# ajaayc/Probability-of-Collision-for-Safe-Planning

Measured on AMD Instinct MI355X. Metric: particle-waypoint evals/s (GMM+collision), higher is better.
Workload: dtype f64

## Files before the change

### probability-of-collision-for-safe-planning_amd/csrc/pocs_collide.h

```cpp
#pragma once
#include "pocs_math.h"

#define POCS_OBS_STRIDE 8
#define POCS_MAX_OBSTACLES 64

struct pocs_footprint { double dx, dy, hx, hy; };

POCS_HD void pocs_prepare_obstacle(const double box5[5], const pocs_footprint* fp, double* rec) {
  double sn, cs;
  pocs_sincos(box5[4], &sn, &cs);
  const double rr = sqrt(fp->hx * fp->hx + fp->hy * fp->hy);
  rec[0] = box5[0]; rec[1] = box5[1];
  rec[2] = cs; rec[3] = sn;
  rec[4] = box5[2]; rec[5] = box5[3];
  rec[6] = (box5[2] * fabs(cs) + box5[3] * fabs(sn)) + rr;
  rec[7] = (box5[2] * fabs(sn) + box5[3] * fabs(cs)) + rr;
}

POCS_HD bool pocs_box_margins(double dx, double dy, double sn, double cs, double rx, double ry, double hx, double hy,
                              double cr, double sr, double e1, double e2) {
  const double m3 = fabs(e1) - (hx + fma(rx, fabs(cr), ry * fabs(sr)));
  const double m4 = fabs(e2) - (hy + fma(rx, fabs(sr), ry * fabs(cr)));
  if (fmax(m3, m4) > 0.0) return false;
#if defined(__HIP_DEVICE_COMPILE__)
  asm volatile("; footprint axes");
#endif
  const double d1 = fma(dx, cs, dy * sn);
  const double d2 = fma(dy, cs, -(dx * sn));
  const double m1 = fabs(d1) - (rx + fma(hx, fabs(cr), hy * fabs(sr)));
  const double m2 = fabs(d2) - (ry + fma(hx, fabs(sr), hy * fabs(cr)));
  return !(fmax(m1, m2) > 0.0);
}

POCS_HD bool pocs_box_narrow(double px, double py, double sn, double cs, double rx, double ry,
                             const double* o) {
  const double dx = o[0] - px;
  const double dy = o[1] - py;
  const double ax = o[2], ay = o[3], hx = o[4], hy = o[5];
  if (ax == 1.0 && ay == 0.0)
    return pocs_box_margins(dx, dy, sn, cs, rx, ry, hx, hy, cs, sn, dx, dy);
  return pocs_box_margins(dx, dy, sn, cs, rx, ry, hx, hy,
                          fma(cs, ax, sn * ay),
                          fma(sn, ax, -(cs * ay)),
                          fma(dx, ax, dy * ay),
                          fma(dy, ax, -(dx * ay)));
}

POCS_HD bool pocs_box_hit(double px, double py, double sn, double cs, double rx, double ry,
                          const double* o) {
  if (fabs(o[0] - px) > o[6] || fabs(o[1] - py) > o[7]) return false;
  return pocs_box_narrow(px, py, sn, cs, rx, ry, o);
}

POCS_HD bool pocs_pose_collides(double x, double y, double th, const pocs_footprint* fp,
                                const double* obs, int M, const pocs_tables* T, const pocs_vconst* V = nullptr) {
  if (M <= 0) return false;
  double sn, cs;
  pocs_sincos_tab(th, T, &sn, &cs, V);
  double px = x, py = y;
  if (!(fp->dx == 0.0 && fp->dy == 0.0)) {
#if defined(__HIP_DEVICE_COMPILE__)
    asm volatile("; offset footprint");
#endif
    px = x + fma(cs, fp->dx, -(sn * fp->dy));
    py = y + fma(sn, fp->dx, cs * fp->dy);
  }
  bool hit = false;
  for (int m = 0; m < M; ++m)
    if (pocs_box_hit(px, py, sn, cs, fp->hx, fp->hy, obs + m * POCS_OBS_STRIDE)) hit = true;
  return hit;
}

template <bool EAGER = false>
POCS_HD void pocs_pair_collides(const double x[2], const double y[2], const double th[2], const pocs_footprint* fp,
                                const double* obs, int M, const pocs_tables* T, const pocs_vconst* V, bool hit[2]) {
  hit[0] = false; hit[1] = false;
  if (M <= 0) return;
  double sn[2], cs[2], px[2], py[2];
#if defined(__HIP_DEVICE_COMPILE__)
#pragma unroll
#endif
  for (int h = 0; h < 2; ++h) {
    pocs_sincos_tab(th[h], T, &sn[h], &cs[h], V);
    px[h] = x[h]; py[h] = y[h];
  }
  if (!(fp->dx == 0.0 && fp->dy == 0.0)) {
#if defined(__HIP_DEVICE_COMPILE__)
    asm volatile("; offset footprint");
#endif
    for (int h = 0; h < 2; ++h) {
      px[h] = x[h] + fma(cs[h], fp->dx, -(sn[h] * fp->dy));
      py[h] = y[h] + fma(sn[h], fp->dx, cs[h] * fp->dy);
    }
  }
  for (int m = 0; m < M; ++m) {
    const double* o = obs + m * POCS_OBS_STRIDE;
#if defined(__HIP_DEVICE_COMPILE__)
    double rec[POCS_OBS_STRIDE];
    if (EAGER) {
#pragma unroll
      for (int q = 0; q < POCS_OBS_STRIDE; ++q) rec[q] = o[q];
      asm volatile("" : "+v"(rec[0]), "+v"(rec[1]), "+v"(rec[2]), "+v"(rec[3]), "+v"(rec[4]), "+v"(rec[5]), "+v"(rec[6]), "+v"(rec[7]));
      o = rec;
    }
#pragma unroll
#endif
    for (int h = 0; h < 2; ++h)
      if (pocs_box_hit(px[h], py[h], sn[h], cs[h], fp->hx, fp->hy, o)) hit[h] = true;
  }
}

template <class Each>
POCS_HD bool pocs_pose_collides_each(double x, double y, double th, const pocs_footprint* fp, const double* obs, int M,
                                     const pocs_tables* T, Each each, const pocs_vconst* V = nullptr) {
  if (M <= 0) return false;
  double sn, cs;
  pocs_sincos_tab(th, T, &sn, &cs, V);
  double px = x, py = y;
  if (!(fp->dx == 0.0 && fp->dy == 0.0)) {
#if defined(__HIP_DEVICE_COMPILE__)
    asm volatile("; offset footprint");
#endif
    px = x + fma(cs, fp->dx, -(sn * fp->dy));
    py = y + fma(sn, fp->dx, cs * fp->dy);
  }
  bool hit = false;
  for (int m = 0; m < M; ++m) {
    const bool t = pocs_box_hit(px, py, sn, cs, fp->hx, fp->hy, obs + m * POCS_OBS_STRIDE);
    if (t) hit = true;
    each(m, t);
  }
  return hit;
}

template <bool EAGER = false, class Each>
POCS_HD void pocs_pair_collides_each(const double x[2], const double y[2], const double th[2], const pocs_footprint* fp,
                                     const double* obs, int M, const pocs_tables* T, const pocs_vconst* V, bool hit[2], Each each) {
  hit[0] = false; hit[1] = false;
  if (M <= 0) return;
  double sn[2], cs[2], px[2], py[2];
#if defined(__HIP_DEVICE_COMPILE__)
#pragma unroll
#endif
  for (int h = 0; h < 2; ++h) {
    pocs_sincos_tab(th[h], T, &sn[h], &cs[h], V);
    px[h] = x[h]; py[h] = y[h];
  }
  if (!(fp->dx == 0.0 && fp->dy == 0.0)) {
#if defined(__HIP_DEVICE_COMPILE__)
    asm volatile("; offset footprint");
#endif
    for (int h = 0; h < 2; ++h) {
      px[h] = x[h] + fma(cs[h], fp->dx, -(sn[h] * fp->dy));
      py[h] = y[h] + fma(sn[h], fp->dx, cs[h] * fp->dy);
    }
  }
  for (int m = 0; m < M; ++m) {
    const double* o = obs + m * POCS_OBS_STRIDE;
#if defined(__HIP_DEVICE_COMPILE__)
    double rec[POCS_OBS_STRIDE];
    if (EAGER) {
#pragma unroll
      for (int q = 0; q < POCS_OBS_STRIDE; ++q) rec[q] = o[q];
      asm volatile("" : "+v"(rec[0]), "+v"(rec[1]), "+v"(rec[2]), "+v"(rec[3]), "+v"(rec[4]), "+v"(rec[5]), "+v"(rec[6]), "+v"(rec[7]));
      o = rec;
    }
#pragma unroll
#endif
    for (int h = 0; h < 2; ++h) {
      const bool t = pocs_box_hit(px[h], py[h], sn[h], cs[h], fp->hx, fp->hy, o);
      if (t) hit[h] = true;
      each(m, h, t);
    }
  }
}

POCS_HD bool pocs_footprint_extent_is_radius(double phi, double lo, double hi) {
  const double PI = 3.14159265358979323846, INV_PI = 0.318309886183790671538;
  if (!(hi - lo < PI)) return true;
  for (int sgn = -1; sgn <= 1; sgn += 2) {
    const double s = sgn * phi;
    if (ceil((lo - s) * INV_PI) <= floor((hi - s) * INV_PI)) return true;
  }
  return false;
}
POCS_HD double pocs_footprint_extent_end(double rx, double ry, double t) {
  double sn, cs;
  pocs_sincos(t, &sn, &cs);
  return fma(rx, fabs(cs), ry * fabs(sn));
}
POCS_HD double pocs_footprint_extent_of_ends(double rr, double fa, double fb) {
  return fmin(rr, fmax(fa, fb) * (1.0 + 1e-9) + 1e-12);
}
POCS_HD double pocs_footprint_extent_pre(double rx, double ry, double rr, double phi, double lo, double hi) {
  if (pocs_footprint_extent_is_radius(phi, lo, hi)) return rr;
  const double fa = pocs_footprint_extent_end(rx, ry, lo);
  const double fb = pocs_footprint_extent_end(rx, ry, hi);
  return pocs_footprint_extent_of_ends(rr, fa, fb);
}
POCS_HD double pocs_footprint_extent(double rx, double ry, double lo, double hi) {
  return pocs_footprint_extent_pre(rx, ry, sqrt(rx * rx + ry * ry), atan2(ry, rx), lo, hi);
}
```

### probability-of-collision-for-safe-planning_amd/csrc/pocs_dev_gmm.hpp

```cpp

template <bool OC> struct gmm_oc_smem {};
template <> struct gmm_oc_smem<true> {
  unsigned occ[2][POCS_MAX_OBSTACLES];
  int oci[2][POCS_MAX_OBSTACLES];
};
template <int K, int TB, bool OC = false>
struct gmm_smem : gmm_oc_smem<OC> {
  static constexpr int NC = K * POCS_NMOM;
  static constexpr int NW = TB / 64;
  static constexpr int SUB = POCS_GMM_SUB;
  alignas(16) pocs_tables tab;
  alignas(16) double keep[2][POCS_MAX_OBSTACLES * POCS_OBS_STRIDE];
  alignas(16) double par[2][K * POCS_PARAM_STRIDE];
  alignas(16) double tr[NW][POCS_FLUSH_ROWS][POCS_FLUSH_PITCH];
  alignas(16) double slot[SUB][NW][POCS_UNIT_SUMS];
  double xtra[2][NW][K][POCS_UNIT_SUMS];
  int kf[SUB][NW];
  int xj[2][NW][K];
  unsigned long long seed[2];
  int nkeep[2];
  int last[2];
  static_assert(sizeof(double) * NW * POCS_FLUSH_ROWS * POCS_FLUSH_PITCH >= sizeof(double) * POCS_MAX_OBSTACLES * POCS_OBS_STRIDE,
                "the obstacle table is staged in the transpose scratch");
  static_assert(NW * POCS_FLUSH_ROWS * POCS_FLUSH_PITCH >= 16 * NC, "the closer's staging rows live in the transpose scratch");
  static_assert(SUB * NW * POCS_UNIT_SUMS >= POCS_ADV_SCRATCH(K) + POCS_SPEC_SCRATCH(K), "the advance's scratch lives in the slots");
  __device__ __forceinline__ double* obs() { return &tr[0][0][0]; }
  __device__ __forceinline__ double* stage() { return &tr[0][0][0]; }
  __device__ __forceinline__ double* adv() { return &slot[0][0][0]; }
  __device__ __forceinline__ double* spec() { return &slot[0][0][0] + POCS_ADV_SCRATCH(K); }
};

__device__ __forceinline__ double oct_sum(double s) {
  s += dpp_f64<0xB1>(s);
  s += dpp_f64<0x4E>(s);
  s += dpp_f64<0x141>(s);
  return s;
}

template <int K, int TB, bool OC>
__device__ __forceinline__ void flush_unit(gmm_smem<K, TB, OC>& sm, const int wave, const int lane, const int rb, const int tl,
                                           const int k, bool& first, double (&acc)[9], int& nfree) {
  double* const T = &sm.tr[wave][0][0];
  double* const dst = first ? &sm.slot[tl][wave][0] : &sm.xtra[rb][wave][k][0];
  const int j = lane >> 3, q = lane & 7;
#pragma unroll
  for (int pass = 0; pass < 2; ++pass) {
    const int nv = pass == 0 ? 5 : 4, v0 = pass == 0 ? 0 : 5;
#pragma unroll
    for (int i = 0; i < nv; ++i) T[i * POCS_FLUSH_PITCH + lane] = acc[v0 + i];
    __builtin_amdgcn_fence(__ATOMIC_RELEASE, "wavefront");
    __builtin_amdgcn_wave_barrier();
    double s = 0.0;
    if (j < nv) {
      const double* p = &T[j * POCS_FLUSH_PITCH + 8 * q];
      s = p[0]; s += p[1]; s += p[2]; s += p[3]; s += p[4]; s += p[5]; s += p[6]; s += p[7];
    }
    s = oct_sum(s);
    if (j < nv && q == 0) dst[1 + v0 + j] = s;
    __builtin_amdgcn_fence(__ATOMIC_RELEASE, "wavefront");
    __builtin_amdgcn_wave_barrier();
  }
  if (lane == 0) {
    dst[0] = (double)nfree;
    if (first) sm.kf[tl][wave] = k; else sm.xj[rb][wave][k] = tl;
  }
#pragma unroll
  for (int i = 0; i < 9; ++i) acc[i] = 0.0;
  nfree = 0;
  first = false;
}

template <int K>
__device__ __forceinline__ void gmm_reach(const pocs_footprint& fp, const double fp_rr, const double fp_phi, const int lane, const double* par,
                                          pocs_reach& rc, double& ext_x, double& ext_y) {
  pocs_world_reach_box(par, K, fp, rc);
  const double tlo = rc.tlo, thi = rc.thi;
  const double HALF_PI = 1.57079632679489661923;
  const double end_t = ((lane & 1) ? thi : tlo) - ((lane & 2) ? HALF_PI : 0.0);
  const double end_f = pocs_footprint_extent_end(fp.hx, fp.hy, end_t);
  ext_x = pocs_footprint_extent_is_radius(fp_phi, tlo, thi) ? fp_rr
        : pocs_footprint_extent_of_ends(fp_rr, lane_value(end_f, 0), lane_value(end_f, 1));
  ext_y = pocs_footprint_extent_is_radius(fp_phi, tlo - HALF_PI, thi - HALF_PI) ? fp_rr
        : pocs_footprint_extent_of_ends(fp_rr, lane_value(end_f, 2), lane_value(end_f, 3));
}
template <int K, int TB, bool OC>
__device__ __forceinline__ void gmm_cull(const pocs_gmm_launch& a, gmm_smem<K, TB, OC>& sm, const int rb, const int lane, const double* par) {
  const pocs_footprint fp = a.fp;
  const int M = a.M;
  const double* const obs = sm.obs();
  double xlo = 1e300, xhi = -1e300, ylo = 1e300, yhi = -1e300, tlo = 1e300, thi = -1e300;
#pragma unroll
  for (int k = 0; k < K; ++k) {
    const double* p = &par[k * POCS_PARAM_STRIDE];
    const double ex = 6.67 * fabs(p[3]), ey = 6.67 * (fabs(p[4]) + fabs(p[5])), et = 6.67 * (fabs(p[6]) + fabs(p[7]) + fabs(p[8]));
    xlo = fmin(xlo, p[0] - ex); xhi = fmax(xhi, p[0] + ex);
    ylo = fmin(ylo, p[1] - ey); yhi = fmax(yhi, p[1] + ey);
    tlo = fmin(tlo, p[2] - et); thi = fmax(thi, p[2] + et);
  }
  const double pad = sqrt(fp.dx * fp.dx + fp.dy * fp.dy) + 1e-6;
  xlo -= pad; xhi += pad; ylo -= pad; yhi += pad;
  tlo -= 1e-9 * (1.0 + fabs(tlo)); thi += 1e-9 * (1.0 + fabs(thi));
  const double HALF_PI = 1.57079632679489661923;
  const double end_t = ((lane & 1) ? thi : tlo) - ((lane & 2) ? HALF_PI : 0.0);
  const double end_f = pocs_footprint_extent_end(fp.hx, fp.hy, end_t);
  const double ext_x = pocs_footprint_extent_is_radius(a.fp_phi, tlo, thi) ? a.fp_rr
                     : pocs_footprint_extent_of_ends(a.fp_rr, lane_value(end_f, 0), lane_value(end_f, 1));
  const double ext_y = pocs_footprint_extent_is_radius(a.fp_phi, tlo - HALF_PI, thi - HALF_PI) ? a.fp_rr
                     : pocs_footprint_extent_of_ends(a.fp_rr, lane_value(end_f, 2), lane_value(end_f, 3));
  bool keep = false;
  double bx = 0.0, by = 0.0;
  if (lane < M) {
    const double* o = &obs[lane * POCS_OBS_STRIDE];
    bx = fmin(o[6], fma(o[4], fabs(o[2]), o[5] * fabs(o[3])) * (1.0 + 1e-12) + ext_x);
    by = fmin(o[7], fma(o[4], fabs(o[3]), o[5] * fabs(o[2])) * (1.0 + 1e-12) + ext_y);
    keep = !(o[0] - bx > xhi || o[0] + bx < xlo || o[1] - by > yhi || o[1] + by < ylo);
  }
  const unsigned long long mask = __ballot(keep);
  if (keep) {
    const int pos = __popcll(mask & ((1ull << lane) - 1ull));
#pragma unroll
    for (int j = 0; j < 6; ++j) sm.keep[rb][pos * POCS_OBS_STRIDE + j] = obs[lane * POCS_OBS_STRIDE + j];
    sm.keep[rb][pos * POCS_OBS_STRIDE + 6] = bx;
    sm.keep[rb][pos * POCS_OBS_STRIDE + 7] = by;
    if constexpr (OC) sm.oci[rb][pos] = lane;
  }
  if constexpr (OC) sm.occ[rb][lane] = 0u;
  if (lane == 0) sm.nkeep[rb] = __popcll(mask);
}

template <int K, bool STORE, int TB, bool LONE_PRE = false, bool OC = false>
__device__ __forceinline__ void gmm_units(const pocs_gmm_launch& a, gmm_smem<K, TB, OC>& sm, const int w, const int r0,
                                          const int ta, const int tb, const double* zpre = nullptr, const int npre = 0) {
  const pocs_tables* const s_tab = &sm.tab;
  const int tid = threadIdx.x, lane = tid & 63;
  const int wave = __builtin_amdgcn_readfirstlane(tid >> 6);
  const pocs_footprint fp = a.fp;
  const int vs_mask = (1 << a.vs_shift) - 1;
  double acc[9];
  int nfree = 0;
#pragma unroll
  for (int j = 0; j < 9; ++j) acc[j] = 0.0;
  const int count = (int)a.count;
  const int npairs = (count + 1) >> 1;
  const uint64_t pair0 = (uint64_t)(a.first >> 1);
  const double first_d = (double)a.first;
  const int wave_first = 128 * wave;
  const int prio_slot = (TB >= 512 ? (wave >> 2) : 0) + (TB >= 512 ? 2 : 1) * (int)((blockIdx.x >> 8) & 3u);
  int prio_it = prio_slot;
  int rb = -1, nkeep = 0, kcur = 0, kw = 0;
  const double* s_par = nullptr;
  const double* s_keep = nullptr;
  uint64_t seed = 0;
  double cumn[K > 1 ? K - 1 : 1];
  double *xr = nullptr, *yr = nullptr, *tr = nullptr;
  int16_t* fr = nullptr;
  int seg_end = 0;
  POCS_VCONST(vc_);
  const pocs_vconst* const vc = &vc_;

  int it_unit = 0;
  auto iteration = [&](auto whole_tag, const int base, const int tl, bool& first) __attribute__((always_inline)) {
    constexpr bool WHOLE = decltype(whole_tag)::value;
    switch (prio_it++ & 3) {
      case 0: __builtin_amdgcn_s_setprio(0); break;
      case 1: __builtin_amdgcn_s_setprio(1); break;
      case 2: __builtin_amdgcn_s_setprio(2); break;
      default: __builtin_amdgcn_s_setprio(3); break;
    }
    const int lp = base + tid;
    const bool live = WHOLE || lp < npairs;
    double zz[2][3];
    uint32_t spare[2];
    uint64_t seed_it = seed;
#if defined(__HIP_DEVICE_COMPILE__)
    asm volatile("" : "+s"(seed_it));
#endif
    bool drawn = false;
    if constexpr (LONE_PRE) {
      if (it_unit < npre) {
        const double* z = zpre + (size_t)it_unit * 6 * TB + tid;
#pragma unroll
        for (int q = 0; q < 3; ++q) { zz[0][q] = z[q * TB]; zz[1][q] = z[(3 + q) * TB]; }
        drawn = true;
        ++it_unit;
      }
    }
    if (!drawn) {
      POCS_TUNE_NORMALS(pocs_normal3_pair(seed_it, pair0 + (uint64_t)(unsigned)lp, (uint32_t)w, POCS_STREAM_GMM, s_tab, zz[0], zz[1], &spare[0], &spare[1], vc));
    }
    const int i0 = 2 * lp;
    const bool two = WHOLE || (live && (i0 + 1) < count);
    double xs[2], ys[2], ts[2];
    bool hits[2];
    int ks[2];
#pragma unroll
    for (int h = 0; h < 2; ++h) {
      int k = kw;
      if (!WHOLE) {
        const double gidx = (first_d + (double)i0) + (double)h;
        k = 0;
#pragma unroll
        for (int j = 0; j < K - 1; ++j) k += (cumn[j] <= gidx) ? 1 : 0;
      }
      const double* p = &s_par[k * POCS_PARAM_STRIDE];
      xs[h] = fma(p[3], zz[h][0], p[0]);
      ys[h] = fma(p[5], zz[h][1], fma(p[4], zz[h][0], p[1]));
      ts[h] = fma(p[8], zz[h][2], fma(p[7], zz[h][1], fma(p[6], zz[h][0], p[2])));
      ks[h] = k;
    }
    POCS_TUNE_COLLIDE_STATS();
    if constexpr (OC) {
      unsigned* const occ = sm.occ[rb];
      pocs_pair_collides_each<LONE_PRE>(xs, ys, ts, &fp, s_keep, nkeep, s_tab, vc, hits, [&](const int m, const int h, const bool t) {
        const unsigned long long b = __ballot(t && (h == 0 ? live : two));
        if (b != 0ull && lane == (int)__builtin_ctzll(b))
          __hip_atomic_fetch_add(&occ[m], (unsigned)__popcll(b), __ATOMIC_RELAXED, __HIP_MEMORY_SCOPE_WORKGROUP);
      });
    } else {
    POCS_TUNE_COLLIDE(pocs_pair_collides<LONE_PRE>(xs, ys, ts, &fp, s_keep, nkeep, s_tab, vc, hits));
    }
    if constexpr (POCS_TUNE_SKIP_MOMENTS) { POCS_TUNE_MOMENTS_ALT(); } else {
    if (WHOLE) {
#pragma unroll
      for (int h = 0; h < 2; ++h) {
        nfree += __popcll(__ballot(!hits[h]));
        if (!hits[h]) {
          const double x = xs[h], y = ys[h], t = ts[h];
          acc[0] += x; acc[1] += y; acc[2] += t;
          acc[3] = fma(x, x, acc[3]); acc[4] = fma(x, y, acc[4]); acc[5] = fma(x, t, acc[5]);
          acc[6] = fma(y, y, acc[6]); acc[7] = fma(y, t, acc[7]); acc[8] = fma(t, t, acc[8]);
        }
      }
    } else {
      const unsigned long long live_mask = __ballot(live);
      const int klo = live_mask ? __builtin_amdgcn_readlane(ks[0], (int)__builtin_ctzll(live_mask)) : K;
      const int khi = __ballot(two) == ~0ull ? __builtin_amdgcn_readlane(ks[1], 63) : K - 1;
#pragma unroll
      for (int kk = 0; kk < K; ++kk) {
        if (kk < klo || kk > khi) continue;
        if (kk != kcur) { flush_unit(sm, wave, lane, rb, tl, kcur, first, acc, nfree); kcur = kk; }
#pragma unroll
        for (int h = 0; h < 2; ++h) {
          const bool sel = (h == 0 ? live : two) && ks[h] == kk;
          const bool cnt = sel && !hits[h];
          nfree += __popcll(__ballot(cnt));
          const double ind = cnt ? 1.0 : 0.0;
          const double xm = ind * xs[h], ym = ind * ys[h], tm = ind * ts[h];
          acc[0] += xm; acc[1] += ym; acc[2] += tm;
          acc[3] = fma(xm, xs[h], acc[3]); acc[4] = fma(xm, ys[h], acc[4]); acc[5] = fma(xm, ts[h], acc[5]);
          acc[6] = fma(ym, ys[h], acc[6]); acc[7] = fma(ym, ts[h], acc[7]); acc[8] = fma(tm, ts[h], acc[8]);
        }
      }
    }
    }
    if (STORE && live) {
      const size_t ub = 2 * (size_t)(unsigned)base;
      const int fl = (hits[0] ? 1 : 0) | ((two && hits[1]) ? 0x10000 : 0);
      store16_nt(xr + ub, 16u * (unsigned)tid, (v2d){xs[0], xs[1]});
      store16_nt(yr + ub, 16u * (unsigned)tid, (v2d){ys[0], ys[1]});
      store16_nt(tr + ub, 16u * (unsigned)tid, (v2d){ts[0], ts[1]});
      store4_nt(fr + ub, 4u * (unsigned)tid, fl);
    }
  };

  auto lookup = [&](const int l0) __attribute__((always_inline)) {
    const double g0 = first_d + (double)l0;
    int kk = 0;
#pragma unroll
    for (int q = 0; q < K - 1; ++q) kk += (cumn[q] <= g0) ? 1 : 0;
    kw = __builtin_amdgcn_readfirstlane(kk);
    double e = (double)count;
    if (kw < K - 1) e = fmin(e, s_par[kw * POCS_PARAM_STRIDE + 9] - first_d);
    seg_end = __builtin_amdgcn_readfirstlane((int)e);
  };
  for (int t = ta; t < tb; ++t) {
    const int tl = t - ta;
    const int r = t >> a.vs_shift, j = t & vs_mask;
    if (r - r0 != rb) {
      rb = r - r0;
      s_par = sm.par[rb]; s_keep = sm.keep[rb];
      nkeep = __builtin_amdgcn_readfirstlane(sm.nkeep[rb]);
      seed = (uint64_t)uniform64((long long)sm.seed[rb]);
#pragma unroll
      for (int q = 0; q < K - 1; ++q) cumn[q] = s_par[q * POCS_PARAM_STRIDE + 9];
      xr = a.x + (size_t)r * a.sample_stride;
      yr = a.y + (size_t)r * a.sample_stride;
      tr = a.th + (size_t)r * a.sample_stride;
      fr = a.flags + (size_t)r * a.sample_stride;
      seg_end = 0;
    }
    const int c_begin = (int)(((long long)j * a.chunks) >> a.vs_shift);
    const int c_end = (int)(((long long)(j + 1) * a.chunks) >> a.vs_shift);
    bool first = true;
    it_unit = (t == ta) ? 0 : npre;
    const int end = c_end * TB;
    int base = c_begin * TB;
    if (2 * base + wave_first + 128 > seg_end) lookup(2 * base + wave_first);
    kcur = kw;
    while (base < end) {
      int l0 = 2 * base + wave_first;
      if (l0 + 128 > seg_end) lookup(l0);
      if (l0 + 128 <= seg_end) {
        if (kw != kcur) { flush_unit(sm, wave, lane, rb, tl, kcur, first, acc, nfree); kcur = kw; }
        do {
          iteration(std::true_type{}, base, tl, first);
          base += TB;
          l0 += 2 * TB;
        } while (base < end && l0 + 128 <= seg_end);
      } else {
        iteration(std::false_type{}, base, tl, first);
        base += TB;
      }
    }
    __builtin_amdgcn_s_setprio(3);
    flush_unit(sm, wave, lane, rb, tl, kcur, first, acc, nfree);
  }
}

template <int K, int TB, bool OC>
__device__ __forceinline__ void gmm_emit_rows(const pocs_gmm_launch& a, gmm_smem<K, TB, OC>& sm, const int r0, const int ta, const int tb) {
  constexpr int NC = K * POCS_NMOM, NW = TB / 64;
  for (int i = threadIdx.x; i < (tb - ta) * NC; i += TB) {
    const int tl = i / NC, c = i - tl * NC, k = c / POCS_NMOM, col = c - k * POCS_NMOM;
    const int rb = ((ta + tl) >> a.vs_shift) - r0;
    double v = 0.0;
    if (col != 1) {
      const int s = col == 0 ? 0 : col - 1;
      double ps[NW], px[NW];
      int kf[NW], xj[NW];
#pragma unroll
      for (int u = 0; u < NW; ++u) { kf[u] = sm.kf[tl][u]; xj[u] = sm.xj[rb][u][k]; ps[u] = sm.slot[tl][u][s]; px[u] = sm.xtra[rb][u][k][s]; }
#pragma unroll
      for (int u = 0; u < NW; ++u) {
        const double p = kf[u] == k ? ps[u] : (xj[u] == tl ? px[u] : 0.0);
        v = (u == 0) ? p : v + p;
      }
    }
    store_wt(&a.partial[(size_t)(ta + tl) * NC + c], v);
  }
}

template <int K, int NT>
struct close_rows {
  static constexpr int NC = K * POCS_NMOM, G = 16, ITEMS = G * NC, RPI = POCS_GMM_MAX_VS / G;
  double v[2][RPI];
  __device__ __forceinline__ void request(const double* src, const int S, const int i0) {
#pragma unroll
    for (int t = 0; t < 2; ++t) {
      const int i = i0 + t * NT, g = i / NC, c = i - g * NC;
#pragma unroll
      for (int u = 0; u < RPI; ++u) {
        const int q = g + u * G;
        v[t][u] = (i < ITEMS && q < S) ? load_wt(&src[(size_t)q * NC + c]) : 0.0;
      }
    }
  }
  __device__ __forceinline__ void pin() {
    static_assert(RPI % 4 == 0, "four values per statement");
#pragma unroll
    for (int t = 0; t < 2; ++t)
#pragma unroll
      for (int u = 0; u < RPI; u += 4) asm volatile("" : "+v"(v[t][u]), "+v"(v[t][u + 1]), "+v"(v[t][u + 2]), "+v"(v[t][u + 3]));
  }
  __device__ __forceinline__ void reduce(double* stage, const int S, const int i0) const {
#pragma unroll
    for (int t = 0; t < 2; ++t) {
      const int i = i0 + t * NT, g = i / NC;
      double sum = 0.0;
#pragma unroll
      for (int u = 0; u < RPI; ++u) if (g + u * G < S) sum += v[t][u];
      if (i < ITEMS) stage[i] = sum;
    }
  }
};
template <int K>
__device__ __forceinline__ const double* close_rows_of(const pocs_gmm_launch& a, const double* rows, const int r) {
  return rows + (size_t)r * (1 << a.vs_shift) * (K * POCS_NMOM);
}
template <int K, int NT, bool REQUESTED = false>
__device__ __forceinline__ void gmm_close_sums(const pocs_gmm_launch& a, const int w, const int r, const double* s_par,
                                               double* stage, double* tot, const int tid,
                                               const double* rows, const bool store, close_rows<K, NT>& cr) {
  constexpr int NC = K * POCS_NMOM, G = 16, ITEMS = G * NC, nthreads = NT;
  const int S = 1 << a.vs_shift;
  const double* src = close_rows_of<K>(a, rows, r);
  for (int i0 = tid; i0 < ITEMS; i0 += 2 * NT) {
    if (!(REQUESTED && i0 == tid)) cr.request(src, S, i0);
    requests_issued();
    cr.pin();
    cr.reduce(stage, S, i0);
  }
  __syncthreads();
  for (int c = tid; c < NC; c += nthreads) {
    double v = stage[c];
    const int ng = S < G ? S : G;
    for (int g = 1; g < ng; ++g) v += stage[g * NC + c];
    tot[c] = v;
  }
  __syncthreads();
  const double lo = (double)a.first, hi = (double)(a.first + a.count);
  for (int k = tid; k < K; k += nthreads) {
    const double c0 = (k == 0) ? 0.0 : s_par[(k - 1) * POCS_PARAM_STRIDE + 9];
    const double c1 = (k == K - 1) ? (double)a.n_total : s_par[k * POCS_PARAM_STRIDE + 9];
    const double n_k = fmax(0.0, fmin(c1, hi) - fmax(c0, lo));
    tot[k * POCS_NMOM + 1] = n_k - tot[k * POCS_NMOM];
  }
  __syncthreads();
  if (store) for (int c = tid; c < NC; c += nthreads) a.moments[((size_t)w * a.nruns + r) * NC + c] = tot[c];
}

template <int K, bool STORE, int TB, bool LONE, bool RISK, bool TREE = false, bool OC = false, bool WORLD = false>
__device__ __forceinline__ void gmm_step_block(const pocs_gmm_launch a) {
  typedef gmm_smem<K, TB, OC> smem_t;
  static_assert(!(WORLD && (LONE || TREE || OC)), "a large world: the ticket form of a batch or of plans, no per-box counts");
  static_assert(!WORLD || TB == POCS_MAX_OBSTACLES * POCS_OBS_STRIDE, "one element of a run's kept records per thread");
  static_assert(!(LONE && RISK), "the lone form closes in its heads: a call under a risk bound takes the ticket form");
  static_assert(!(TREE && (LONE || STORE)), "a tree's levels take the ticket form and store no samples");
  constexpr int SUB = smem_t::SUB, NW = smem_t::NW;
  __shared__ smem_t sm;
  __shared__ double s_zpre[LONE ? POCS_LONE_PRE * 6 * TB : 2];
  int npre = 0;
  const int tid = threadIdx.x;
  const int w = a.waypoint;
  const int wr = TREE ? 0 : w;
  const int t_lo = a.run_lo << a.vs_shift, t_hi = (a.run_lo + a.run_cnt) << a.vs_shift;
  const int bx = (int)blockIdx.x;
  const int t0_all = t_lo + bx * a.upb;
  const int t1_all = (t0_all + a.upb < t_hi) ? t0_all + a.upb : t_hi;
  const int r0_all = t0_all >> a.vs_shift, r1_all = (t1_all - 1) >> a.vs_shift;
  int t0 = t0_all, t1 = t1_all, r0 = r0_all, r1 = r1_all;
  POCS_STAMP_BEGIN();
  constexpr int PS = K * POCS_PARAM_STRIDE;
  static_assert(POCS_MAX_OBSTACLES * POCS_OBS_STRIDE <= TB, "one obstacle element per thread");
  static_assert(2 * PS <= TB, "one sampler parameter per thread (two runs)");
  static_assert(POCS_ADV_STAGE_MAX <= 4 * TB, "the advance's inputs in one batch");
  double tabv[table_regs<TB>::N];
  request_tables<TB>(a.tables, tid, tabv);
  double obs_elem = 0.0;
  if constexpr (!WORLD) obs_elem = tid < a.M * POCS_OBS_STRIDE ? a.env->obs[tid] : 0.0;
  if (LONE && w > 0) {
    const bool out = blockIdx.x == 0;
    const adv_ptrs ap = advance_ptrs(a, K, w, r0, sm.adv());
    double advv[4];
    advance_request(ap, false, tid, TB, advv);
    const double parv = tid < PS ? a.param[((size_t)r0 * a.W + (w - 1)) * PS + tid] : 0.0;
    const unsigned long long seedv = a.hdr[r0].seed;
    close_rows<K, TB> cr;
    cr.request(close_rows_of<K>(a, a.partial_prev, r0), 1 << a.vs_shift, tid);
    requests_issued();
    commit_tables<TB>(&sm.tab, tid, tabv);
    advance_commit(ap, false, tid, TB, advv);
    if (tid < PS) sm.par[1][tid] = parv;
    for (int j = tid; j < 2 * NW * K; j += TB) (&sm.xj[0][0][0])[j] = -1;
    if (tid == 0) sm.seed[0] = seedv;
    double* const l_mom = ap.l_mom;
    gmm_close_sums<K, TB, true>(a, w - 1, r0, sm.par[1], sm.stage(), l_mom, tid, a.partial_prev, out, cr);
    POCS_STAMP(5);
    if (tid < a.M * POCS_OBS_STRIDE) sm.obs()[tid] = obs_elem;
    const int j0 = t0 & ((1 << a.vs_shift) - 1);
    const int cb0 = (int)(((long long)j0 * a.chunks) >> a.vs_shift), ce0 = (int)(((long long)(j0 + 1) * a.chunks) >> a.vs_shift);
    npre = (ce0 - cb0) < POCS_LONE_PRE ? (ce0 - cb0) : POCS_LONE_PRE;
    auto draw_ahead = [&]() __attribute__((always_inline)) {
      POCS_VCONST(vc_);
      const uint64_t seed = seedv;
      const uint64_t pair0 = (uint64_t)(a.first >> 1);
      for (int it = 0; it < npre; ++it)
        for (int l = tid - 128; l < TB; l += TB - 128) {
          double za[3], zb[3];
          uint32_t sa, sb;
          pocs_normal3_pair(seed, pair0 + (uint64_t)(unsigned)((cb0 + it) * TB + l), (uint32_t)w, POCS_STREAM_GMM, &sm.tab, za, zb, &sa, &sb, &vc_);
          double* z = s_zpre + (size_t)it * 6 * TB + l;
#pragma unroll
          for (int q = 0; q < 3; ++q) { z[q * TB] = za[q]; z[(3 + q) * TB] = zb[q]; }
        }
    };
    auto cull_early = [&]() __attribute__((always_inline)) { gmm_cull(a, sm, 0, tid - 64, ap.l_par); };
    if (tid < 128) __builtin_amdgcn_s_setprio(3);
    advance_block(a, K, w, r0, sm.adv(), sm.spec(), true, tid, TB, true, out, draw_ahead, cull_early);
    if (tid < 128) __builtin_amdgcn_s_setprio(0);
    __syncthreads();
    POCS_STAMP(6);
    POCS_STAMP_COUNT(14);
    const double* const l_par = advance_ptrs(a, K, w, r0, sm.adv()).l_par;
    for (int j = tid; j < PS; j += TB) sm.par[0][j] = l_par[j];
  } else {
    const int rp = tid / PS, jp = tid - rp * PS;
    const double parv = tid < (r1 - r0 + 1) * PS ? load_wt(&a.param[((size_t)(r0 + rp) * a.W + wr) * PS + jp]) : 0.0;
    const unsigned long long seedv = tid <= r1 - r0 ? a.hdr[r0 + tid].seed : 0ull;
    double keptv[2] = {0.0, 0.0};
    int reachv[2] = {0, 0};
    if constexpr (WORLD) {
#pragma unroll
      for (int q = 0; q < 2; ++q) {
        const int rq = r0_all + q <= r1_all ? r0_all + q : r1_all;
        keptv[q] = load_wt(&a.kept[(size_t)rq * (POCS_MAX_OBSTACLES * POCS_OBS_STRIDE) + tid]);
        reachv[q] = __hip_atomic_load(&a.reach[(size_t)rq * a.W + wr], __ATOMIC_RELAXED, __HIP_MEMORY_SCOPE_AGENT);
      }
    }
    auto commit_world = [&](const int shift) __attribute__((always_inline)) {
      if constexpr (WORLD) {
#pragma unroll
        for (int q = 0; q < 2; ++q) {
          const int rb = q - shift;
          if (q <= r1_all - r0_all && rb >= 0 && rb <= r1 - r0) {
            const int n = reachv[q] < POCS_MAX_OBSTACLES ? reachv[q] : POCS_MAX_OBSTACLES;
            if (tid < n * POCS_OBS_STRIDE) sm.keep[rb][tid] = keptv[q];
            if (tid == 0) sm.nkeep[rb] = n;
          }
        }
      }
    };
    if constexpr (RISK) {
      const unsigned s0 = __hip_atomic_load(&a.stop[r0_all], __ATOMIC_RELAXED, __HIP_MEMORY_SCOPE_AGENT);
      const unsigned s1 = __hip_atomic_load(&a.stop[r1_all], __ATOMIC_RELAXED, __HIP_MEMORY_SCOPE_AGENT);
      requests_issued();
      const bool dead0 = __builtin_amdgcn_readfirstlane((int)s0) != 0, dead1 = __builtin_amdgcn_readfirstlane((int)s1) != 0;
      if (dead0 && dead1) return;
      int shift = 0;
      if (dead0) { shift = 1; r0 = r1_all; t0 = r1_all << a.vs_shift; }
      else if (dead1) { r1 = r0_all; t1 = r1_all << a.vs_shift; }
      commit_tables<TB>(&sm.tab, tid, tabv);
      if (tid < a.M * POCS_OBS_STRIDE) sm.obs()[tid] = obs_elem;
      if (tid < (r1_all - r0_all + 1) * PS && rp >= shift && rp - shift <= r1 - r0) sm.par[rp - shift][jp] = parv;
      for (int j = tid; j < 2 * NW * K; j += TB) (&sm.xj[0][0][0])[j] = -1;
      if (tid <= r1_all - r0_all && tid >= shift && tid - shift <= r1 - r0) sm.seed[tid - shift] = seedv;
      commit_world(shift);
    } else {
    requests_issued();
    commit_tables<TB>(&sm.tab, tid, tabv);
    if (tid < a.M * POCS_OBS_STRIDE) sm.obs()[tid] = obs_elem;
    if (tid < (r1 - r0 + 1) * PS) sm.par[rp][jp] = parv;
    for (int j = tid; j < 2 * NW * K; j += TB) (&sm.xj[0][0][0])[j] = -1;
    if (tid <= r1 - r0) sm.seed[tid] = seedv;
    commit_world(0);
    }
  }
  __syncthreads();
  if constexpr (!WORLD) {
  if (!(LONE && w > 0)) {
    if (tid < 64) gmm_cull(a, sm, 0, tid, sm.par[0]);
    else if (tid < 128 && r1 > r0) gmm_cull(a, sm, 1, tid - 64, sm.par[1]);
    __syncthreads();
  }
  }
  POCS_STAMP(0);
  for (int ta = t0; ta < t1; ta += SUB) {
    const int tb = (ta + SUB < t1) ? ta + SUB : t1;
    gmm_units<K, STORE, TB, LONE, OC>(a, sm, w, r0, ta, tb, s_zpre, ta == t0 ? npre : 0);
    POCS_STAMP(1);
    __syncthreads();
    POCS_STAMP(2);
    gmm_emit_rows(a, sm, r0, ta, tb);
    if (tb < t1) {
      __syncthreads();
      for (int j = tid; j < 2 * NW * K; j += TB) (&sm.xj[0][0][0])[j] = -1;
      __syncthreads();
    }
  }
  if constexpr (OC) {
    const int rb = tid >> 6, j = tid & 63;
// ... 196 lines not shown
```

### probability-of-collision-for-safe-planning_amd/csrc/pocs_tuning.h

```cpp
#ifndef POCS_TUNING_HOOKS
#define POCS_TUNING_HOOKS

#if defined(POCS_STAMPS)
__device__ unsigned long long g_stamps[24 * 256];
#define POCS_STAMP_AT(i) (&g_stamps[(i) + 24 * (blockIdx.x & 255)])
#define POCS_STAMP_BEGIN() unsigned long long last_ = wall_clock64(); if (threadIdx.x == 0) atomicAdd(POCS_STAMP_AT(15), 1ull)
#define POCS_STAMP(i) do { if (threadIdx.x == 0) { const unsigned long long n_ = wall_clock64(); atomicAdd(POCS_STAMP_AT(i), n_ - last_); last_ = n_; } } while (0)
#define POCS_STAMP_COUNT(i) do { if (threadIdx.x == 0) atomicAdd(POCS_STAMP_AT(i), 1ull); } while (0)
#define POCS_ADV_STAMP_BEGIN() unsigned long long t_ = wall_clock64()
#define POCS_ADV_STAMP(i) do { if (tid == 0) { const unsigned long long n_ = wall_clock64(); atomicAdd(POCS_STAMP_AT(i), n_ - t_); t_ = n_; } } while (0)
#define POCS_TUNE_COLLIDE_STATS() do { bool pass_ = false; \
    for (int m_ = 0; m_ < nkeep; ++m_) { const double* o_ = s_keep + m_ * POCS_OBS_STRIDE; \
      for (int h_ = 0; h_ < 2; ++h_) pass_ = pass_ || (fabs(o_[0] - xs[h_]) <= o_[6] && fabs(o_[1] - ys[h_]) <= o_[7]); } \
    const unsigned long long b_ = __ballot(pass_); \
    bool own_ = false; { const double* p_ = &s_par[ks[0] * POCS_PARAM_STRIDE]; const double ex_ = 6.67 * fabs(p_[3]), ey_ = 6.67 * (fabs(p_[4]) + fabs(p_[5])); \
      for (int m_ = 0; m_ < nkeep; ++m_) { const double* o_ = s_keep + m_ * POCS_OBS_STRIDE; \
        own_ = own_ || (fabs(o_[0] - p_[0]) <= o_[6] + ex_ && fabs(o_[1] - p_[1]) <= o_[7] + ey_); } } \
    const unsigned long long c_ = __ballot(own_); \
    if ((threadIdx.x & 63) == 0) { atomicAdd(POCS_STAMP_AT(16), 1ull); if (nkeep > 0) atomicAdd(POCS_STAMP_AT(17), 1ull); if (b_) atomicAdd(POCS_STAMP_AT(18), 1ull); \
      atomicAdd(POCS_STAMP_AT(19), (unsigned long long)nkeep); atomicAdd(POCS_STAMP_AT(20), (unsigned long long)__popcll(b_)); if (c_ & 1ull) atomicAdd(POCS_STAMP_AT(21), 1ull); } } while (0)
#else
#define POCS_TUNE_COLLIDE_STATS() do { } while (0)
#define POCS_STAMP_BEGIN() do { } while (0)
#define POCS_STAMP(i) do { } while (0)
#define POCS_STAMP_COUNT(i) do { } while (0)
#define POCS_ADV_STAMP_BEGIN() do { } while (0)
#define POCS_ADV_STAMP(i) do { } while (0)
#endif

#if defined(POCS_ABLATE_RNG)
#define POCS_TUNE_NORMALS(...) for (int h = 0; h < 2; ++h) { zz[h][0] = (double)(lp & 7) * 0.1; zz[h][1] = (double)(lp & 3) * 0.1; zz[h][2] = 0.05; spare[h] = (uint32_t)lp * 2654435761u; }
#elif defined(POCS_ABLATE_PHILOX)
#define POCS_TUNE_NORMALS(...) { const uint32_t q = (uint32_t)(pair0 + lp) * 2654435761u ^ (uint32_t)seed ^ ((uint32_t)w << 20); \
      const uint32_t a0 = q * 0x9E3779B1u, a1 = (q ^ 0x85EBCA6Bu) * 0xC2B2AE35u, a2 = (q + 0x27D4EB2Fu) * 0x165667B1u; \
      pocs_normal_pair_w2(a0, a1, s_tab, &zz[0][0], &zz[0][1]); \
      pocs_normal_pair_w2(a2, a0 ^ a1, s_tab, &zz[0][2], &zz[1][0]); \
      pocs_normal_pair_w2(a1 ^ a2, a0 + a2, s_tab, &zz[1][1], &zz[1][2]); \
      spare[0] = a0; spare[1] = a1; }
#elif defined(POCS_ABLATE_BOXMULLER)
#define POCS_TUNE_NORMALS(...) { const pocs_u32x4 A = pocs_draw(seed, pair0 + lp, (uint32_t)w, POCS_STREAM_GMM, 0u), B = pocs_draw(seed, pair0 + lp, (uint32_t)w, POCS_STREAM_GMM, 1u); \
      zz[0][0] = (double)A.x * 0x1p-32; zz[0][1] = (double)A.y * 0x1p-32; zz[0][2] = (double)A.z * 0x1p-32; spare[0] = B.z; \
      zz[1][0] = (double)A.w * 0x1p-32; zz[1][1] = (double)B.x * 0x1p-32; zz[1][2] = (double)B.y * 0x1p-32; spare[1] = B.w; }
#else
#define POCS_TUNE_NORMALS(...) __VA_ARGS__
#endif
#if defined(POCS_ABLATE_COLLIDE)
#define POCS_TUNE_COLLIDE(...) hits[0] = xs[0] > ts[0]; hits[1] = xs[1] > ts[1]
#else
#define POCS_TUNE_COLLIDE(...) __VA_ARGS__
#endif
#if defined(POCS_ABLATE_MOMENTS)
#define POCS_TUNE_SKIP_MOMENTS true
#define POCS_TUNE_MOMENTS_ALT() do { acc[1] += xs[0] + ys[0] + ts[0] + xs[1]; nfree += (hits[0] || (two && ks[1] == 0)) ? 0 : 1; } while (0)
#else
#define POCS_TUNE_SKIP_MOMENTS false
#define POCS_TUNE_MOMENTS_ALT() do { } while (0)
#endif

#endif

#if defined(POCS_STAMPS) && defined(POCS_TUNING_REPORT)
extern "C" void pocs_stamps_report() {
  static unsigned long long all[24 * 256];
  unsigned long long h[24] = {0};
  if (hipMemcpyFromSymbol(all, HIP_SYMBOL(g_stamps), sizeof all) != hipSuccess) return;
  for (int b = 0; b < 256; ++b) for (int i = 0; i < 24; ++i) h[i] += all[24 * b + i];
  if (h[15] == 0) return;
  const double nb = (double)h[15], nc = (double)(h[14] ? h[14] : 1);
  fprintf(stderr, "[stamps] %.0f blocks, %.0f closers; per block (us): head %.2f | units %.2f | -> barrier %.2f | rows + drain + barrier %.2f | "
          "ticket + barrier %.2f ; per closer: close_sums %.2f | advance %.2f (staging %.2f, components (wave 0) %.2f, -> the counts lane %.2f, normalise + publish + drain %.2f)\n",
          nb, nc, 0.01 * h[0] / nb, 0.01 * h[1] / nb, 0.01 * h[2] / nb, 0.01 * h[3] / nb, 0.01 * h[4] / nb, 0.01 * h[5] / nc, 0.01 * h[6] / nc,
          0.01 * h[8] / nc, 0.01 * h[9] / nc, 0.01 * h[10] / nc, 0.01 * h[11] / nc);
  if (h[16]) fprintf(stderr, "[stamps] footprint test: %llu wave iterations, %.1f %% in runs with kept records (%.2f records per iteration), %.1f %% with a lane inside a record's broad-phase box (%.2f lanes per iteration); %.1f %% where the box of the wave's OWN component (first lane's) reaches a kept record\n",
                     h[16], 100.0 * h[17] / h[16], (double)h[19] / h[16], 100.0 * h[18] / h[16], (double)h[20] / h[16], 100.0 * h[21] / h[16]);
  for (auto& v : all) v = 0;
  (void)hipMemcpyToSymbol(HIP_SYMBOL(g_stamps), all, sizeof all);
}
#endif
```

Baseline: 167.9 billion.

## Rewrite pair collision test with wave-wide ballot masks and lazy heading evaluation

The per-lane collision loop for particle pairs becomes a wave-uniform loop that builds 64-bit ballot masks. A whole wave skips the narrow phase for an obstacle when no lane passes the broad phase. For centred footprints, the sincos of the heading is deferred until some lane first reaches an obstacle's broad box. Obstacle records are read as paired-double vectors from LDS with precomputed footprint extents, and hit results are carried as masks through the moments and store code. This aims to cut divergent branches and redundant trig and extent work, at the cost of more complex mask plumbing and assumptions about the address space and wave64.

After: 173.2 billion, median of 6. 1.03x the previous value.

```diff
diff --git a/probability-of-collision-for-safe-planning_amd/csrc/pocs_collide.h b/probability-of-collision-for-safe-planning_amd/csrc/pocs_collide.h
--- a/probability-of-collision-for-safe-planning_amd/csrc/pocs_collide.h
+++ b/probability-of-collision-for-safe-planning_amd/csrc/pocs_collide.h
@@ -71,23 +71,125 @@
   return hit;
 }
 
+#if defined(__HIPCC__)
+typedef double pocs_v2d __attribute__((ext_vector_type(2)));
+struct pocs_each_none { __device__ __forceinline__ void operator()(int, int, bool) const {} };
+
+__device__ __forceinline__ unsigned long long pocs_box_margins_mask(unsigned long long pm, double dx, double dy, double sn, double cs,
+                                                                    double rx, double ry, double hx, double hy,
+                                                                    double cr, double sr, double e1, double e2,
+                                                                    double p3, double p4) {
+  const double m3 = fabs(e1) - (hx + p3);
+  const double m4 = fabs(e2) - (hy + p4);
+  const unsigned long long near = pm & __builtin_amdgcn_ballot_w64(!(fmax(m3, m4) > 0.0));
+  if (near == 0ull) return 0ull;
+  asm volatile("; footprint axes");
+  const double d1 = fma(dx, cs, dy * sn);
+  const double d2 = fma(dy, cs, -(dx * sn));
+  const double m1 = fabs(d1) - (rx + fma(hx, fabs(cr), hy * fabs(sr)));
+  const double m2 = fabs(d2) - (ry + fma(hx, fabs(sr), hy * fabs(cr)));
+  return near & __builtin_amdgcn_ballot_w64(!(fmax(m1, m2) > 0.0));
+}
+
+template <bool EAGER, bool CENTRED, class Each>
+__device__ __forceinline__ void pocs_pair_loop(const double x[2], const double y[2], const double th[2], const pocs_footprint* fp,
+                                               const double* obs, int M, const pocs_tables* T, const pocs_vconst* V,
+                                               unsigned long long mask[2], Each each) {
+  const double rx = fp->hx, ry = fp->hy;
+  double sn[2], cs[2], px[2], py[2];
+  double ex[2], ey[2];
+  bool heading = false;
+  if (CENTRED) asm volatile("" : "=v"(sn[0]), "=v"(cs[0]), "=v"(sn[1]), "=v"(cs[1]), "=v"(ex[0]), "=v"(ey[0]), "=v"(ex[1]), "=v"(ey[1]));
+  if (!CENTRED) {
+#pragma unroll
+    for (int h = 0; h < 2; ++h) {
+      pocs_sincos_tab(th[h], T, &sn[h], &cs[h], V);
+      px[h] = x[h] + fma(cs[h], fp->dx, -(sn[h] * fp->dy));
+      py[h] = y[h] + fma(sn[h], fp->dx, cs[h] * fp->dy);
+      ex[h] = fma(rx, fabs(cs[h]), ry * fabs(sn[h]));
+      ey[h] = fma(rx, fabs(sn[h]), ry * fabs(cs[h]));
+    }
+    heading = true;
+  }
+  unsigned long long m0 = 0ull, m1 = 0ull;
+  const __attribute__((address_space(3))) pocs_v2d* o = (const __attribute__((address_space(3))) pocs_v2d*)obs;
+  asm volatile("" : "+v"(o));
+  for (int m = 0; m < M; ++m, o += POCS_OBS_STRIDE / 2) {
+    pocs_v2d c = o[0], b = o[3], a = o[1], e = o[2];
+    if (EAGER) asm volatile("" : "+v"(c), "+v"(b), "+v"(a), "+v"(e));
+    double dx[2], dy[2];
+    unsigned long long pm[2], bt[2] = {0ull, 0ull};
+#pragma unroll
+    for (int h = 0; h < 2; ++h) {
+      dx[h] = c.x - (CENTRED ? x[h] : px[h]);
+      dy[h] = c.y - (CENTRED ? y[h] : py[h]);
+      pm[h] = __builtin_amdgcn_ballot_w64(!(fabs(dx[h]) > b.x)) & __builtin_amdgcn_ballot_w64(!(fabs(dy[h]) > b.y));
+    }
+    if ((pm[0] | pm[1]) != 0ull) {
+      if (CENTRED && !heading) {
+#pragma unroll
+        for (int h = 0; h < 2; ++h) {
+          double t = th[h];
+          asm volatile("" : "+v"(t));
+          pocs_sincos_tab(t, T, &sn[h], &cs[h], V);
+          ex[h] = fma(rx, fabs(cs[h]), ry * fabs(sn[h]));
+          ey[h] = fma(rx, fabs(sn[h]), ry * fabs(cs[h]));
+        }
+        heading = true;
+      }
+      const bool turned = (__builtin_amdgcn_ballot_w64(a.x != 1.0) | __builtin_amdgcn_ballot_w64(a.y != 0.0)) != 0ull;
+#pragma unroll
+      for (int h = 0; h < 2; ++h) {
+        if (pm[h] == 0ull) continue;
+        if (!turned)
+          bt[h] = pocs_box_margins_mask(pm[h], dx[h], dy[h], sn[h], cs[h], rx, ry, e.x, e.y, cs[h], sn[h], dx[h], dy[h], ex[h], ey[h]);
+        else {
+          const double cr = fma(cs[h], a.x, sn[h] * a.y), sr = fma(sn[h], a.x, -(cs[h] * a.y));
+          bt[h] = pocs_box_margins_mask(pm[h], dx[h], dy[h], sn[h], cs[h], rx, ry, e.x, e.y, cr, sr,
+                                        fma(dx[h], a.x, dy[h] * a.y), fma(dy[h], a.x, -(dx[h] * a.y)),
+                                        fma(rx, fabs(cr), ry * fabs(sr)), fma(rx, fabs(sr), ry * fabs(cr)));
+        }
+      }
+      m0 |= bt[0]; m1 |= bt[1];
+    }
+#pragma unroll
+    for (int h = 0; h < 2; ++h) each(m, h, __builtin_amdgcn_inverse_ballot_w64(bt[h]));
+  }
+  mask[0] = m0; mask[1] = m1;
+}
+
+template <bool EAGER = false, class Each = pocs_each_none>
+__device__ __forceinline__ void pocs_pair_collides_masks(const double x[2], const double y[2], const double th[2], const pocs_footprint* fp,
+                                                         const double* obs, int M, const pocs_tables* T, const pocs_vconst* V,
+                                                         unsigned long long mask[2], Each each = Each()) {
+  mask[0] = 0ull; mask[1] = 0ull;
+  if (M <= 0) return;
+  if (fp->dx == 0.0 && fp->dy == 0.0) {
+    pocs_pair_loop<EAGER, true>(x, y, th, fp, obs, M, T, V, mask, each);
+  } else {
+    asm volatile("; offset footprint");
+    pocs_pair_loop<EAGER, false>(x, y, th, fp, obs, M, T, V, mask, each);
+  }
+}
+#endif
+
 template <bool EAGER = false>
 POCS_HD void pocs_pair_collides(const double x[2], const double y[2], const double th[2], const pocs_footprint* fp,
                                 const double* obs, int M, const pocs_tables* T, const pocs_vconst* V, bool hit[2]) {
+#if defined(__HIP_DEVICE_COMPILE__)
+  unsigned long long mask[2];
+  pocs_pair_collides_masks<EAGER>(x, y, th, fp, obs, M, T, V, mask);
+  hit[0] = __builtin_amdgcn_inverse_ballot_w64(mask[0]);
+  hit[1] = __builtin_amdgcn_inverse_ballot_w64(mask[1]);
+#else
   hit[0] = false; hit[1] = false;
   if (M <= 0) return;
   double sn[2], cs[2], px[2], py[2];
-#if defined(__HIP_DEVICE_COMPILE__)
-#pragma unroll
-#endif
   for (int h = 0; h < 2; ++h) {
     pocs_sincos_tab(th[h], T, &sn[h], &cs[h], V);
     px[h] = x[h]; py[h] = y[h];
   }
   if (!(fp->dx == 0.0 && fp->dy == 0.0)) {
-#if defined(__HIP_DEVICE_COMPILE__)
-    asm volatile("; offset footprint");
-#endif
     for (int h = 0; h < 2; ++h) {
       px[h] = x[h] + fma(cs[h], fp->dx, -(sn[h] * fp->dy));
       py[h] = y[h] + fma(sn[h], fp->dx, cs[h] * fp->dy);
@@ -95,19 +197,10 @@
   }
   for (int m = 0; m < M; ++m) {
     const double* o = obs + m * POCS_OBS_STRIDE;
-#if defined(__HIP_DEVICE_COMPILE__)
-    double rec[POCS_OBS_STRIDE];
-    if (EAGER) {
-#pragma unroll
-      for (int q = 0; q < POCS_OBS_STRIDE; ++q) rec[q] = o[q];
-      asm volatile("" : "+v"(rec[0]), "+v"(rec[1]), "+v"(rec[2]), "+v"(rec[3]), "+v"(rec[4]), "+v"(rec[5]), "+v"(rec[6]), "+v"(rec[7]));
-      o = rec;
-    }
-#pragma unroll
-#endif
     for (int h = 0; h < 2; ++h)
       if (pocs_box_hit(px[h], py[h], sn[h], cs[h], fp->hx, fp->hy, o)) hit[h] = true;
   }
+#endif
 }
 
 template <class Each>
@@ -136,20 +229,20 @@
 template <bool EAGER = false, class Each>
 POCS_HD void pocs_pair_collides_each(const double x[2], const double y[2], const double th[2], const pocs_footprint* fp,
                                      const double* obs, int M, const pocs_tables* T, const pocs_vconst* V, bool hit[2], Each each) {
+#if defined(__HIP_DEVICE_COMPILE__)
+  unsigned long long mask[2];
+  pocs_pair_collides_masks<EAGER>(x, y, th, fp, obs, M, T, V, mask, each);
+  hit[0] = __builtin_amdgcn_inverse_ballot_w64(mask[0]);
+  hit[1] = __builtin_amdgcn_inverse_ballot_w64(mask[1]);
+#else
   hit[0] = false; hit[1] = false;
   if (M <= 0) return;
   double sn[2], cs[2], px[2], py[2];
-#if defined(__HIP_DEVICE_COMPILE__)
-#pragma unroll
-#endif
   for (int h = 0; h < 2; ++h) {
     pocs_sincos_tab(th[h], T, &sn[h], &cs[h], V);
     px[h] = x[h]; py[h] = y[h];
   }
   if (!(fp->dx == 0.0 && fp->dy == 0.0)) {
-#if defined(__HIP_DEVICE_COMPILE__)
-    asm volatile("; offset footprint");
-#endif
     for (int h = 0; h < 2; ++h) {
       px[h] = x[h] + fma(cs[h], fp->dx, -(sn[h] * fp->dy));
       py[h] = y[h] + fma(sn[h], fp->dx, cs[h] * fp->dy);
@@ -157,22 +250,13 @@
   }
   for (int m = 0; m < M; ++m) {
     const double* o = obs + m * POCS_OBS_STRIDE;
-#if defined(__HIP_DEVICE_COMPILE__)
-    double rec[POCS_OBS_STRIDE];
-    if (EAGER) {
-#pragma unroll
-      for (int q = 0; q < POCS_OBS_STRIDE; ++q) rec[q] = o[q];
-      asm volatile("" : "+v"(rec[0]), "+v"(rec[1]), "+v"(rec[2]), "+v"(rec[3]), "+v"(rec[4]), "+v"(rec[5]), "+v"(rec[6]), "+v"(rec[7]));
-      o = rec;
-    }
-#pragma unroll
-#endif
     for (int h = 0; h < 2; ++h) {
       const bool t = pocs_box_hit(px[h], py[h], sn[h], cs[h], fp->hx, fp->hy, o);
       if (t) hit[h] = true;
       each(m, h, t);
     }
   }
+#endif
 }
 
 POCS_HD bool pocs_footprint_extent_is_radius(double phi, double lo, double hi) {
diff --git a/probability-of-collision-for-safe-planning_amd/csrc/pocs_dev_gmm.hpp b/probability-of-collision-for-safe-planning_amd/csrc/pocs_dev_gmm.hpp
--- a/probability-of-collision-for-safe-planning_amd/csrc/pocs_dev_gmm.hpp
+++ b/probability-of-collision-for-safe-planning_amd/csrc/pocs_dev_gmm.hpp
@@ -191,7 +191,7 @@
     const int i0 = 2 * lp;
     const bool two = WHOLE || (live && (i0 + 1) < count);
     double xs[2], ys[2], ts[2];
-    bool hits[2];
+    unsigned long long hits[2];
     int ks[2];
 #pragma unroll
     for (int h = 0; h < 2; ++h) {
@@ -211,20 +211,20 @@
     POCS_TUNE_COLLIDE_STATS();
     if constexpr (OC) {
       unsigned* const occ = sm.occ[rb];
-      pocs_pair_collides_each<LONE_PRE>(xs, ys, ts, &fp, s_keep, nkeep, s_tab, vc, hits, [&](const int m, const int h, const bool t) {
+      pocs_pair_collides_masks<LONE_PRE>(xs, ys, ts, &fp, s_keep, nkeep, s_tab, vc, hits, [&](const int m, const int h, const bool t) {
         const unsigned long long b = __ballot(t && (h == 0 ? live : two));
         if (b != 0ull && lane == (int)__builtin_ctzll(b))
           __hip_atomic_fetch_add(&occ[m], (unsigned)__popcll(b), __ATOMIC_RELAXED, __HIP_MEMORY_SCOPE_WORKGROUP);
       });
     } else {
-    POCS_TUNE_COLLIDE(pocs_pair_collides<LONE_PRE>(xs, ys, ts, &fp, s_keep, nkeep, s_tab, vc, hits));
+    POCS_TUNE_COLLIDE(pocs_pair_collides_masks<LONE_PRE>(xs, ys, ts, &fp, s_keep, nkeep, s_tab, vc, hits));
     }
     if constexpr (POCS_TUNE_SKIP_MOMENTS) { POCS_TUNE_MOMENTS_ALT(); } else {
     if (WHOLE) {
 #pragma unroll
       for (int h = 0; h < 2; ++h) {
-        nfree += __popcll(__ballot(!hits[h]));
-        if (!hits[h]) {
+        nfree += __popcll(~hits[h]);
+        if (!__builtin_amdgcn_inverse_ballot_w64(hits[h])) {
           const double x = xs[h], y = ys[h], t = ts[h];
           acc[0] += x; acc[1] += y; acc[2] += t;
           acc[3] = fma(x, x, acc[3]); acc[4] = fma(x, y, acc[4]); acc[5] = fma(x, t, acc[5]);
@@ -242,7 +242,7 @@
 #pragma unroll
         for (int h = 0; h < 2; ++h) {
           const bool sel = (h == 0 ? live : two) && ks[h] == kk;
-          const bool cnt = sel && !hits[h];
+          const bool cnt = sel && !__builtin_amdgcn_inverse_ballot_w64(hits[h]);
           nfree += __popcll(__ballot(cnt));
           const double ind = cnt ? 1.0 : 0.0;
           const double xm = ind * xs[h], ym = ind * ys[h], tm = ind * ts[h];
@@ -255,7 +255,8 @@
     }
     if (STORE && live) {
       const size_t ub = 2 * (size_t)(unsigned)base;
-      const int fl = (hits[0] ? 1 : 0) | ((two && hits[1]) ? 0x10000 : 0);
+      const int fl = (__builtin_amdgcn_inverse_ballot_w64(hits[0]) ? 1 : 0) |
+                     ((two && __builtin_amdgcn_inverse_ballot_w64(hits[1])) ? 0x10000 : 0);
       store16_nt(xr + ub, 16u * (unsigned)tid, (v2d){xs[0], xs[1]});
       store16_nt(yr + ub, 16u * (unsigned)tid, (v2d){ys[0], ys[1]});
       store16_nt(tr + ub, 16u * (unsigned)tid, (v2d){ts[0], ts[1]});
diff --git a/probability-of-collision-for-safe-planning_amd/csrc/pocs_tuning.h b/probability-of-collision-for-safe-planning_amd/csrc/pocs_tuning.h
--- a/probability-of-collision-for-safe-planning_amd/csrc/pocs_tuning.h
+++ b/probability-of-collision-for-safe-planning_amd/csrc/pocs_tuning.h
@@ -45,13 +45,13 @@
 #define POCS_TUNE_NORMALS(...) __VA_ARGS__
 #endif
 #if defined(POCS_ABLATE_COLLIDE)
-#define POCS_TUNE_COLLIDE(...) hits[0] = xs[0] > ts[0]; hits[1] = xs[1] > ts[1]
+#define POCS_TUNE_COLLIDE(...) hits[0] = __ballot(xs[0] > ts[0]); hits[1] = __ballot(xs[1] > ts[1])
 #else
 #define POCS_TUNE_COLLIDE(...) __VA_ARGS__
 #endif
 #if defined(POCS_ABLATE_MOMENTS)
 #define POCS_TUNE_SKIP_MOMENTS true
-#define POCS_TUNE_MOMENTS_ALT() do { acc[1] += xs[0] + ys[0] + ts[0] + xs[1]; nfree += (hits[0] || (two && ks[1] == 0)) ? 0 : 1; } while (0)
+#define POCS_TUNE_MOMENTS_ALT() do { acc[1] += xs[0] + ys[0] + ts[0] + xs[1]; nfree += (__builtin_amdgcn_inverse_ballot_w64(hits[0]) || (two && ks[1] == 0)) ? 0 : 1; } while (0)
 #else
 #define POCS_TUNE_SKIP_MOMENTS false
 #define POCS_TUNE_MOMENTS_ALT() do { } while (0)
```
